# LariWa/Fractal-Image-Compression

Hardware: NVIDIA B200
Metric: encode_evals_per_s (higher is better)
Workload: dtype u8

## Files before the change

### fractal-image-compression_b200/csrc/fic_search_umma.cu

```cuda
#include <cuda_fp16.h>

#include <cmath>
#include <mutex>
#include <tuple>
#include <vector>

#include "fic_device.cuh"

namespace fic {

namespace {

constexpr int kTileN = 128;
constexpr int kBlockM = 128;
constexpr int kAccs = 4;
constexpr int kRowsPerSB = kBlockM * kAccs;
constexpr int kEpiWarps = 16;
constexpr int kThreads = (4 + kEpiWarps) * 32;
constexpr int kChunksPerTile = kTileN / 32;
constexpr int kBoundBytes = kChunksPerTile * 2 * 4 + 16 + kChunksPerTile * 4;
constexpr int kNormOff = kChunksPerTile * 2 * 4 + 16;
constexpr int kFlagLists = 2;
constexpr int kFlagCap = 32;
constexpr float kOneMinusEps = 1.0f - 1.9073486328125e-06f;

template <int B, bool F16>
struct Cfg;
template <>
struct Cfg<8, false> {
    static constexpr int n = 64;
    static constexpr int NB = 4;
    static constexpr bool KSPLIT = false;
    static constexpr int KS_A = 3;
    static constexpr int KS_B = 5;
    static constexpr int NS = 5;
    static constexpr int NSTAGE = 7;
    __host__ __device__ static constexpr int amap(int s) { return s < 4 ? (s & 1) : 2; }
    __host__ __device__ static constexpr bool is_l_slice(int s) { return s == 2 || s == 3; }
// ... 782 lines not shown
                            ((uint32_t)(kBlockM >> 4) << 24);
constexpr uint32_t kIdescF16 = (1u << 4) | (0u << 7) | (0u << 10) | ((uint32_t)(kTileN >> 3) << 17) |
                               ((uint32_t)(kBlockM >> 4) << 24);
constexpr uint32_t kIdescPair = (2u << 4) | (0u << 7) | (1u << 10) | ((uint32_t)(kTileN >> 3) << 17) |
                                ((uint32_t)((2 * kBlockM) >> 4) << 24);
constexpr uint32_t kIdescF16Pair = (1u << 4) | (0u << 7) | (0u << 10) | ((uint32_t)(kTileN >> 3) << 17) |
                                   ((uint32_t)((2 * kBlockM) >> 4) << 24);


template <int B, bool F16, bool PAIR>
__host__ __device__ constexpr int epi_of() { return (!F16 || B == 16) ? 0 : ((B == 4 || PAIR) ? 3 : 2); }

template <int B, bool F16, bool PAIR, bool DUMP>
__global__ void __launch_bounds__(kThreads, 1)
k_umma_search(const uint8_t *__restrict__ opA, const uint8_t *__restrict__ opB, const int32_t *__restrict__ vRarr,
              const float *__restrict__ nRarr, int2 *__restrict__ flag_list, int32_t *__restrict__ flag_cnt, uint32_t *__restrict__ row_lb, int n_sb,
              int n_chunks, int ntiles, int iso_shift, int64_t rows_padded, int32_t *__restrict__ dump, int64_t dump_ld, volatile int *status)
{
    using C = Cfg<B, F16>;
    using L = Lay<B, F16>;
    static_assert(!PAIR || F16 || C::KSPLIT, "CTA pairs: kind::f16, or the K-split configurations (B = 16)");
    constexpr int EPI = DUMP ? 0 : epi_of<B, F16, PAIR>();
    constexpr int NISS = (PAIR && !C::KSPLIT) ? 2 : 1;
    constexpr int NSTAGE = PAIR ? L::PAIR_STAGES : C::NSTAGE;
    constexpr int SLOT = PAIR ? L::PAIR_SLOT_BYTES : L::SLOT_BYTES;
    extern __shared__ __align__(1024) uint8_t smem_raw[];
    uint8_t *smem = (uint8_t *)(((uintptr_t)smem_raw + 1023) & ~(uintptr_t)1023);
    uint8_t *sA = smem;
    uint8_t *sB = smem + L::A_SB_BYTES;
    uint64_t *bars = (uint64_t *)(sB + C::NSTAGE * L::SLOT_BYTES);
    uint32_t bar0 = smem_u32(bars);
    asm volatile("" : "+r"(bar0));
    auto BAR_B_FULL = [&](int s) { return bar0 + 8u * s; };
    auto BAR_B_EMPTY = [&](int s) { return bar0 + 8u * (NSTAGE + s); };
    auto BAR_T_FULL = [&](int q) { return bar0 + 8u * (2 * NSTAGE + q); };
    auto BAR_T_EMPTY = [&](int q) { return bar0 + 8u * (2 * NSTAGE + kAccs + q); };
    const uint32_t BAR_A_FULL = bar0 + 8u * (2 * NSTAGE + 2 * kAccs);
    const uint32_t BAR_A_EMPTY = BAR_A_FULL + 8u;
    uint32_t *tmem_slot = (uint32_t *)(bars + 2 * NSTAGE + 2 * kAccs + 2);
    const uint32_t s_has_l = bar0 + 400u;
    uint32_t *s_lb = (uint32_t *)((uint8_t *)bars + L::BAR_BYTES);

    const int warp = threadIdx.x >> 5, lane = threadIdx.x & 31;
    const uint32_t rank = PAIR ? cluster_ctarank() : 0u;
    const int u_first = PAIR ? (int)(blockIdx.x >> 1) : (int)blockIdx.x, u_step = PAIR ? (int)(gridDim.x >> 1) : (int)gridDim.x;
    const int n_sbu = PAIR ? (n_sb >> 1) : n_sb;

    if (warp == 1 && lane == 0) {
        const uint32_t both = (PAIR && rank == 0) ? 2u : 1u;
        for (int s = 0; s < NSTAGE; s++) {
            mbar_init(BAR_B_FULL(s), both);
            mbar_init(BAR_B_EMPTY(s), NISS);
        }
        for (int q = 0; q < kAccs; q++) {
            mbar_init(BAR_T_FULL(q), 1);
            mbar_init(BAR_T_EMPTY(q), both * (kEpiWarps / kAccs));
        }
        mbar_init(BAR_A_FULL, both);
        mbar_init(BAR_A_EMPTY, NISS);
        asm volatile("fence.mbarrier_init.release.cluster;" ::: "memory");
    }
    if (warp == 2) {
        if (PAIR) {
            asm volatile("tcgen05.alloc.cta_group::2.sync.aligned.shared::cta.b32 [%0], %1;" ::"r"(smem_u32(tmem_slot)), "r"(512u) : "memory");
            asm volatile("tcgen05.relinquish_alloc_permit.cta_group::2.sync.aligned;" ::: "memory");
        } else {
            asm volatile("tcgen05.alloc.cta_group::1.sync.aligned.shared::cta.b32 [%0], %1;" ::"r"(smem_u32(tmem_slot)), "r"(512u) : "memory");
            asm volatile("tcgen05.relinquish_alloc_permit.cta_group::1.sync.aligned;" ::: "memory");
        }
    }
    tc_fence_before();
    if (PAIR) cluster_sync_all();
    else __syncthreads();
    tc_fence_after();
    const uint32_t tmem_base = *tmem_slot;

    const int n_units = n_sbu * n_chunks;

    if (warp == 0) {
        if (lane == 0) {
            uint32_t stage = 0, phase = 0, a_phase = 0;
            for (int u = u_first; u < n_units; u += u_step) {
                int sb = PAIR ? 2 * (u % n_sbu) + (int)rank : u % n_sbu, ch = u / n_sbu;
                int t0 = (int)((int64_t)ch * ntiles / n_chunks), t1 = (int)((int64_t)(ch + 1) * ntiles / n_chunks);
                mbar_wait(BAR_A_EMPTY, a_phase ^ 1, status, 1);
                mbar_expect_tx(BAR_A_FULL, L::A_SB_BYTES);
                bulk_g2s(smem_u32(sA), opA + (int64_t)sb * L::A_SB_BYTES, L::A_SB_BYTES, BAR_A_FULL);
                for (int t = t0; t < t1; t++) {
                    const uint8_t *blob = opB + (int64_t)t * L::B_TILE_BYTES;
                    if (C::KSPLIT && PAIR) {
                        const uint32_t has_l = __ldg((const uint32_t *)(blob + L::B_OP_BYTES + kChunksPerTile * 8));
                        mbar_wait(BAR_B_EMPTY(stage), phase ^ 1, status, 2);
                        sts_u32(s_has_l + 4u * stage, has_l);
                        mbar_expect_tx(BAR_B_FULL(stage), L::PAIR_P0_BYTES);
                        bulk_g2s(smem_u32(sB + stage * SLOT), blob + rank * L::PAIR_P0_BYTES, L::PAIR_P0_BYTES, BAR_B_FULL(stage));
                        if (++stage == NSTAGE) { stage = 0; phase ^= 1; }
                        if (has_l) {
                            mbar_wait(BAR_B_EMPTY(stage), phase ^ 1, status, 2);
                            mbar_expect_tx(BAR_B_FULL(stage), L::PAIR_P1_BYTES);
// ... 22 lines not shown
                        mbar_expect_tx(BAR_B_FULL(stage), L::B_TILE_BYTES);
                        bulk_g2s(smem_u32(sB + stage * L::SLOT_BYTES), blob, L::B_TILE_BYTES, BAR_B_FULL(stage));
                        if (++stage == NSTAGE) { stage = 0; phase ^= 1; }
                    }
                }
                a_phase ^= 1;
            }
        }
        __syncwarp();
    } else if (PAIR && (warp == 1 || (warp == 3 && !C::KSPLIT))) {
        if constexpr (PAIR && C::KSPLIT) {
            if (rank == 0) {
                uint32_t stage = 0, phase = 0, a_phase = 0, t_phase = 0;
                const uint32_t elected = elect_one();
                const uint64_t a_desc0 = make_desc(smem_u32(sA), 128, L::SBO_A);
                for (int u = u_first; u < n_units; u += u_step) {
                    int ch = u / n_sbu;
                    int t0 = (int)((int64_t)ch * ntiles / n_chunks), t1 = (int)((int64_t)(ch + 1) * ntiles / n_chunks);
                    mbar_wait(BAR_A_FULL, a_phase, status, 3);
                    for (int t = t0; t < t1; t++) {
                        mbar_wait(BAR_B_FULL(stage), phase, status, 4);
                        tc_fence_after();
                        const uint32_t has_l = lds_volatile_u32(s_has_l + 4u * stage);
                        const uint64_t b0 = make_desc(smem_u32(sB + stage * SLOT), 128, L::SBO_B);
#pragma unroll
                        for (int q = 0; q < C::NB; q++) {
                            mbar_wait(BAR_T_EMPTY(q), ((t_phase >> q) & 1) ^ 1, status, 5);
                            tc_fence_after();
                            if (elected) {
#pragma unroll
                                for (int s = 0; s < L::KS0; s++) {
                                    const uint64_t ad = a_desc0 + (uint64_t)((q * L::A_BLOCK_BYTES + s * 256) >> 4);
                                    if (F16) tc_mma2_f16(tmem_base + q * kTileN, ad, b0 + (uint64_t)((s * 256) >> 4), kIdescF16Pair, s > 0 ? 1u : 0u);
// ... 26 lines not shown
                                __syncwarp();
                            }
                            if (elected) tc_commit2(BAR_B_EMPTY(stage), 3u);
                            __syncwarp();
                            if (++stage == NSTAGE) { stage = 0; phase ^= 1; }
                        }
                    }
                    if (elected) tc_commit2(BAR_A_EMPTY, 3u);
                    __syncwarp();
                    a_phase ^= 1;
                }
            } else {
                if (lane == 0) {
                    uint32_t stage = 0, phase = 0, a_phase = 0;
                    const uint32_t ra_full = mapa_u32(BAR_A_FULL, 0);
                    for (int u = u_first; u < n_units; u += u_step) {
                        int ch = u / n_sbu;
                        int t0 = (int)((int64_t)ch * ntiles / n_chunks), t1 = (int)((int64_t)(ch + 1) * ntiles / n_chunks);
                        mbar_wait(BAR_A_FULL, a_phase, status, 3);
                        mbar_arrive_cluster(ra_full);
                        for (int t = t0; t < t1; t++) {
                            mbar_wait(BAR_B_FULL(stage), phase, status, 4);
                            const uint32_t has_l = lds_volatile_u32(s_has_l + 4u * stage);
                            mbar_arrive_cluster(mapa_u32(BAR_B_FULL(stage), 0));
                            if (++stage == NSTAGE) { stage = 0; phase ^= 1; }
                            if (has_l) {
                                mbar_wait(BAR_B_FULL(stage), phase, status, 4);
                                mbar_arrive_cluster(mapa_u32(BAR_B_FULL(stage), 0));
                                if (++stage == NSTAGE) { stage = 0; phase ^= 1; }
                            }
                        }
                        a_phase ^= 1;
                    }
                }
                __syncwarp();
            }
        } else if constexpr (PAIR) {
            if (rank == 0) {
                const int qi = warp >> 1;
                uint32_t stage = 0, phase = 0, a_phase = 0, t_phase = 0;
                const uint32_t elected = elect_one();
                const uint64_t a_desc0 = make_desc(smem_u32(sA), 128, L::SBO_A);
                const uint64_t b_desc0 = make_desc(smem_u32(sB), 128, L::SBO_B);
                for (int u = u_first; u < n_units; u += u_step) {
                    int ch = u / n_sbu;
                    int t0 = (int)((int64_t)ch * ntiles / n_chunks), t1 = (int)((int64_t)(ch + 1) * ntiles / n_chunks);
                    mbar_wait(BAR_A_FULL, a_phase, status, 3);
                    for (int t = t0; t < t1; t++) {
                        mbar_wait(BAR_B_FULL(stage), phase, status, 4);
                        tc_fence_after();
                        const uint64_t b_desc = b_desc0 + (uint64_t)((stage * SLOT) >> 4);
#pragma unroll
                        for (int k = 0; k < 2; k++) {
                            const int q = qi + 2 * k;
                            mbar_wait(BAR_T_EMPTY(q), ((t_phase >> k) & 1) ^ 1, status, 5);
                            tc_fence_after();
                            if (elected) {
#pragma unroll
                                for (int s = 0; s < C::NS; s++) {
                                    const uint64_t ad = a_desc0 + (uint64_t)((q * L::A_BLOCK_BYTES + C::amap(s) * 256) >> 4);
                                    tc_mma2_f16(tmem_base + q * kTileN, ad, b_desc + (uint64_t)((s * 256) >> 4), kIdescF16Pair, s > 0 ? 1u : 0u);
// ... 2 lines not shown
                                if (k == 1) tc_commit2(BAR_B_EMPTY(stage), 3u);
                            }
                            __syncwarp();
                            t_phase ^= 1u << k;
                        }
                        if (++stage == NSTAGE) { stage = 0; phase ^= 1; }
                    }
                    if (elected) tc_commit2(BAR_A_EMPTY, 3u);
                    __syncwarp();
                    a_phase ^= 1;
                }
            } else if (warp == 1) {
                if (lane == 0) {
                    uint32_t stage = 0, phase = 0, a_phase = 0;
                    const uint32_t ra_full = mapa_u32(BAR_A_FULL, 0);
                    for (int u = u_first; u < n_units; u += u_step) {
                        int ch = u / n_sbu;
                        int t0 = (int)((int64_t)ch * ntiles / n_chunks), t1 = (int)((int64_t)(ch + 1) * ntiles / n_chunks);
                        mbar_wait(BAR_A_FULL, a_phase, status, 3);
                        mbar_arrive_cluster(ra_full);
                        for (int t = t0; t < t1; t++) {
                            mbar_wait(BAR_B_FULL(stage), phase, status, 4);
                            mbar_arrive_cluster(mapa_u32(BAR_B_FULL(stage), 0));
                            if (++stage == NSTAGE) { stage = 0; phase ^= 1; }
                        }
                        a_phase ^= 1;
                    }
                }
                __syncwarp();
            }
        }
    } else if (warp == 1) {
        uint32_t stage = 0, phase = 0, a_phase = 0, t_phase = 0;
        const uint32_t elected = elect_one();
        const uint64_t a_desc0 = make_desc(smem_u32(sA), 128, L::SBO_A);
        const uint64_t b_desc0 = make_desc(smem_u32(sB), 128, L::SBO_B);
        for (int u = u_first; u < n_units; u += u_step) {
            int ch = u / n_sbu;
            int t0 = (int)((int64_t)ch * ntiles / n_chunks), t1 = (int)((int64_t)(ch + 1) * ntiles / n_chunks);
            mbar_wait(BAR_A_FULL, a_phase, status, 3);
            for (int t = t0; t < t1; t++) {
                mbar_wait(BAR_B_FULL(stage), phase, status, 4);
                tc_fence_after();
                const uint32_t has_l = *(volatile const uint32_t *)(sB + stage * L::SLOT_BYTES + L::B_OP_BYTES + kChunksPerTile * 8);
                if (C::KSPLIT) {
                    const uint64_t b0 = make_desc(smem_u32(sB + stage * L::SLOT_BYTES), 128, L::SBO_B);
#pragma unroll
                    for (int q = 0; q < C::NB; q++) {
                        mbar_wait(BAR_T_EMPTY(q), ((t_phase >> q) & 1) ^ 1, status, 5);
                        tc_fence_after();
                        if (elected) {
#pragma unroll
                            for (int s = 0; s < L::KS0; s++) {
                                const uint64_t ad = a_desc0 + (uint64_t)((q * L::A_BLOCK_BYTES + s * 256) >> 4);
// ... 58 lines not shown
            if (elected) tc_commit(BAR_A_EMPTY);
            __syncwarp();
            a_phase ^= 1;
        }
    } else if (warp >= 4) {
        const int e = warp - 4;
        const int lq = e & 3, q = e >> 2;
        const uint32_t ta = tmem_base + ((uint32_t)(lq * 32) << 16) + q * kTileN;
        uint32_t tf_phase = 0;
        const uint32_t bar_hand_back = PAIR ? mapa_u32(BAR_T_EMPTY(q), 0) : BAR_T_EMPTY(q);
        auto hand_back = [&]() {
            if (PAIR) mbar_arrive_cluster(bar_hand_back);
            else mbar_arrive(bar_hand_back);
        };
        constexpr bool SLACK = B == 16 && F16;
        const int n_units_mine = q < C::NB ? n_units : 0;
        for (int u = u_first; u < n_units_mine; u += u_step) {
            int sb = PAIR ? 2 * (u % n_sbu) + (int)rank : u % n_sbu, ch = u / n_sbu;
            int t0 = (int)((int64_t)ch * ntiles / n_chunks), t1 = (int)((int64_t)(ch + 1) * ntiles / n_chunks);
            const int64_t row = (int64_t)sb * L::ROWS_SB + q * kBlockM + lq * 32 + lane;
            const int vR = vRarr[row];
            const float nR = SLACK ? nRarr[row] : 0.0f;
            RowFilter st;
            st.thresh = (vR == 0) ? __int_as_float(0x7f800000) : -1.0f;
            st.lbmax = 0.0f;
            st.cnt = 0;
            const float tie_abs = (float)(vR * vR) * 4.76837158203125e-07f;
            const uint32_t sh_lb = smem_u32(s_lb + q * kBlockM + (((lq * 32 + lane) >> iso_shift) << iso_shift));
            if (iso_shift) {
                sts_u32(sh_lb, 0u);
                __syncwarp();
            }
            if (ch > 0 && vR != 0) {
                const float seed = __uint_as_float(*(volatile const uint32_t *)(row_lb + ((row >> iso_shift) << iso_shift)));
                if (seed > 0.0f) {
                    st.lbmax = seed;
                    st.thresh = flag_threshold(seed, tie_abs);
                }
            }
            int2 *const list0 = flag_list + (((int64_t)ch * rows_padded + row) * kFlagLists) * kFlagCap;
            int cnt0 = 0, cnt1 = 0;
            for (int t = t0; t < t1; t++) {
                const float4 *gb = (const float4 *)(opB + (int64_t)t * L::B_TILE_BYTES + L::B_OP_BYTES);
                const float4 bnd01 = __ldg(gb), bnd23 = __ldg(gb + 1);
                float4 bndn = make_float4(0.0f, 0.0f, 0.0f, 0.0f);
                if (SLACK) bndn = __ldg(gb + 3);
                mbar_wait(BAR_T_FULL(q), tf_phase, status, 7);
                tc_fence_after();
                if (iso_shift) {
                    const float other = __uint_as_float(lds_volatile_u32(sh_lb));
                    if (other > st.lbmax) {
                        st.lbmax = other;
                        st.thresh = flag_threshold(other, tie_abs);
                    }
                }
// ... 106 lines not shown
                            Mu = M + sl;
                            Ml = fmaxf(M - sl, 0.0f);
                        }
                    }
                    const float ub = Mu * rhi;
                    if (ub > st.thresh) {
                        st.cnt = c < 2 ? cnt0 : cnt1;
                        st = flag_chunk(st, Ml * rlo, ub, tie_abs, list0 + (c >> 1) * kFlagCap, t * kChunksPerTile + c, sh_lb, iso_shift ? 1 : 0);
                        if (c < 2) cnt0 = st.cnt;
                        else cnt1 = st.cnt;
                    }
                }
                }
                tf_phase ^= 1;
            }
            flag_cnt[((int64_t)ch * rows_padded + row) * 2] = cnt0;
            flag_cnt[((int64_t)ch * rows_padded + row) * 2 + 1] = cnt1;
            if (st.lbmax > 0.0f) atomicMax(row_lb + ((row >> iso_shift) << iso_shift), __float_as_uint(st.lbmax));
        }
    }

    tc_fence_before();
    if (PAIR) cluster_sync_all();
    else __syncthreads();
    if (warp == 2) {
        tc_fence_after();
        if (PAIR) asm volatile("tcgen05.dealloc.cta_group::2.sync.aligned.b32 %0, %1;" ::"r"(tmem_base), "r"(512u) : "memory");
        else asm volatile("tcgen05.dealloc.cta_group::1.sync.aligned.b32 %0, %1;" ::"r"(tmem_base), "r"(512u) : "memory");
    }
}


// ... 120 lines not shown
    constexpr int n = B * B;
    int kov = 0;
#pragma unroll
    for (int c = 0; c < n / 16; c++) {
        const uint4 d = __ldg((const uint4 *)(pos_raw + raw_offset<n>(pos, c)));
        const uint4 r = *(const uint4 *)(rw + 4 * c);
        kov = dp4a_uu(r.x, d.x, kov);
        kov = dp4a_uu(r.y, d.y, kov);
        kov = dp4a_uu(r.z, d.z, kov);
        kov = dp4a_uu(r.w, d.w, kov);
    }
    return kov - (rmean * dsum + (dsum / n) * vR);
}

template <class F>
__device__ __forceinline__ void for_each_flagged(int lane, int64_t i, int64_t rows_padded, int n_chunks, int64_t npos,
                                                 const int2 *__restrict__ flag_list, const int32_t *__restrict__ flag_cnt,
                                                 float th, F &&consider)
{
    const int n_lists = kFlagLists * n_chunks;
    const int my_cnt = lane < n_lists ? flag_cnt[((int64_t)(lane / kFlagLists) * rows_padded + i) * kFlagLists + (lane % kFlagLists)] : 0;
    const bool overflow = __any_sync(0xffffffffu, my_cnt > kFlagCap);
    if (!overflow) {
        for (int lh = 0; lh < n_lists; lh++) {
            const int cnt = __shfl_sync(0xffffffffu, my_cnt, lh);
            if (cnt == 0) continue;
            const int2 *lst = flag_list + (((int64_t)(lh / kFlagLists) * rows_padded + i) * kFlagLists + (lh % kFlagLists)) * kFlagCap;
            const int2 mine = lane < cnt ? lst[lane] : make_int2(0, 0);
            unsigned live = __ballot_sync(0xffffffffu, lane < cnt && __int_as_float(mine.y) > th);
            while (live) {
                const int e = __ffs(live) - 1;
                live &= live - 1;
                consider((int64_t)__shfl_sync(0xffffffffu, mine.x, e) * 32 + lane);
            }
        }
    } else {
        for (int64_t pos = lane; pos < npos; pos += 32) consider(pos);
    }
}

template <int B>
__global__ void __launch_bounds__(128)
k_umma_refine(const uint8_t *__restrict__ src, const int32_t *__restrict__ rsum, const uint8_t *__restrict__ pos_raw,
              const int4 *__restrict__ pos_info,
              const int2 *__restrict__ flag_list, const int32_t *__restrict__ flag_cnt,
              const uint32_t *__restrict__ row_lb, int n_chunks,
              int64_t rows_padded, int64_t rows, int64_t npos, const int64_t *__restrict__ dom0_pos,
              int32_t *__restrict__ best, Geom g, int64_t j0)
{
    constexpr int n = B * B;
    constexpr int NW = n / 4;
    const int warp = threadIdx.x >> 5, lane = threadIdx.x & 31;
    const int64_t i = (int64_t)blockIdx.x * 4 + warp;
    if (i >= rows) return;
    const int64_t j = j0 + i;
    int rmean;
    const int vR = centred_sum(rsum[j], n, &rmean);
    if (vR == 0) {
        if (lane == 0) best[j] = 0;
        return;
    }
// ... 25 lines not shown
    auto consider = [&](int64_t pos) {
        const int4 pi = __ldg(pos_info + pos);
        const int idx = pi.x;
        if (idx >= 0) {
            const int varD = pi.y;
            const int kov = refine_kov<B>(rw, rmean, vR, pos_raw, pos, pi.z);
            const float ax = varD > 0 ? fabsf((float)kov) * __frsqrt_rn((float)varD) : 0.0f;
            if (ax * (1.0f + 2.384185791015625e-07f) > th) {
                argmin_merge(be, bi, grey_error(kov, vR, __dsqrt_rn((double)varD)), idx);
                const float xlo = ax * (1.0f - 2.384185791015625e-07f);
                if (xlo > lb) { lb = xlo; th = flag_threshold(lb, tie_abs); }
            }
        }
    };
    if (lane == 0) consider(*dom0_pos);
    for_each_flagged(lane, i, rows_padded, n_chunks, npos, flag_list, flag_cnt, th_row, consider);
    warp_argmin(be, bi);
    if (lane == 0) best[j] = bi == 0x7fffffff ? 0 : bi;
}

template <int B>
__global__ void __launch_bounds__(128)
k_umma_refine_iso(const uint8_t *__restrict__ src, const int32_t *__restrict__ rsum, const uint8_t *__restrict__ pos_raw,
                  const int4 *__restrict__ pos_info, const int2 *__restrict__ flag_list,
                  const int32_t *__restrict__ flag_cnt, const uint32_t *__restrict__ row_lb, int n_chunks,
                  int64_t rows_padded, int64_t ranges, int64_t npos,
                  const int64_t *__restrict__ dom0_pos, int32_t *__restrict__ best, Geom g, int64_t j0)
{
    constexpr int n = B * B;
    constexpr int NW = n / 4;
    __shared__ uint8_t s_blk[4][n];
    const int warp = threadIdx.x >> 5, lane = threadIdx.x & 31;
    const int64_t r = (int64_t)blockIdx.x * 4 + warp;
    if (r >= ranges) return;
    const int64_t j = j0 + r;
    int rmean;
    const int vR = centred_sum(rsum[j], n, &rmean);
    if (vR == 0) {
        if (lane == 0) best[j] = 0;
        return;
// ... 28 lines not shown
        const int4 pi = __ldg(pos_info + pos);
        if (pi.x >= 0) {
            const int kov = refine_kov<B>(rw, rmean, vR, pos_raw, pos, pi.z);
            const float ax = pi.y > 0 ? fabsf((float)kov) * __frsqrt_rn((float)pi.y) : 0.0f;
            if (ax * (1.0f + 2.384185791015625e-07f) > th) {
                argmin_merge(be, bi, grey_error(kov, vR, __dsqrt_rn((double)pi.y)), pi.x * 8 + kiso);
                const float xlo = ax * (1.0f - 2.384185791015625e-07f);
                if (xlo > lb) { lb = xlo; th = flag_threshold(lb, tie_abs); }
            }
        }
    };
    build(0);
    if (lane == 0) consider(*dom0_pos, 0);
    int built = 0;
    bool overflow = false;
    for (int ch = 0; ch < n_chunks && !overflow; ch++) {
        const int64_t base = ((int64_t)ch * rows_padded + r * 8) * kFlagLists;
        const int my_cnt = lane < 8 * kFlagLists ? flag_cnt[base + lane] : 0;
        if (__any_sync(0xffffffffu, my_cnt > kFlagCap)) { overflow = true; break; }
        for (int kiso = 0; kiso < 8; kiso++) {
            int any = 0;
            for (int h = 0; h < kFlagLists; h++) any |= __shfl_sync(0xffffffffu, my_cnt, kFlagLists * kiso + h);
            if (any == 0) continue;
            if (built != kiso) { build(kiso); built = kiso; }
#pragma unroll 1
            for (int h = 0; h < kFlagLists; h++) {
                const int cnt = __shfl_sync(0xffffffffu, my_cnt, kFlagLists * kiso + h);
                if (cnt == 0) continue;
                const int2 *lst = flag_list + (base + kFlagLists * kiso + h) * kFlagCap;
                const int2 mine = lane < cnt ? lst[lane] : make_int2(0, 0);
                unsigned live = __ballot_sync(0xffffffffu, lane < cnt && __int_as_float(mine.y) > th_row);
// ... 7 lines not shown
    }
    if (overflow) {
        for (int kiso = 0; kiso < 8; kiso++) {
            build(kiso);
            for (int64_t pos = lane; pos < npos; pos += 32) consider(pos, kiso);
        }
    }
    warp_argmin(be, bi);
    if (lane == 0) best[j] = bi == 0x7fffffff ? 0 : bi;
}

template <int B>
__global__ void __launch_bounds__(128)
k_umma_refine_rgb(const uint8_t *__restrict__ src, const int32_t *__restrict__ rsum, const uint8_t *__restrict__ opB,
                  const int4 *__restrict__ pos_info, const int2 *__restrict__ flag_list, const int32_t *__restrict__ flag_cnt,
                  const uint32_t *__restrict__ row_lb, int n_chunks,
                  int64_t rows_padded, int64_t rows, int64_t npos, const int64_t *__restrict__ dom0_pos,
                  int32_t *__restrict__ best, Geom g, int64_t j0)
{
    using L = Lay<B, true>;
    constexpr int n = B * B;
    const int warp = threadIdx.x >> 5, lane = threadIdx.x & 31;
    const int64_t i = (int64_t)blockIdx.x * 4 + warp;
    if (i >= rows) return;
    const int64_t j = j0 + i;
    int rm[3];
    const int vRi = centred_sum_rgb(rsum, g.NR, j, n, rm);
    const int rmsum = rm[0] + rm[1] + rm[2];
    if (vRi == 0) {
        if (lane == 0) best[j] = 0;
        return;
// ... 29 lines not shown
                    const float2 f = __half22float2(*(const __half2 *)&w[e]);
                    kov = rgb_kov_step(kov, gR[c * 8 + 2 * e], f.x);
                    kov = rgb_kov_step(kov, gR[c * 8 + 2 * e + 1], f.y);
                }
            }
            const float vD = (float)pi.y;
            const float ax = pi.y > 0 ? __fdiv_rn(fabsf(kov), vD) : 0.0f;
            if (ax * (1.0f + 2.384185791015625e-07f) > th) {
                argmin_merge(be, bi, rgb_error(kov, vR, vD), idx);
                const float xlo = ax * (1.0f - 2.384185791015625e-07f);
                if (xlo > lb) { lb = xlo; th = flag_threshold(lb, tie_abs); }
            }
        }
    };
    if (lane == 0) consider(*dom0_pos);
    for_each_flagged(lane, i, rows_padded, n_chunks, npos, flag_list, flag_cnt, th_row, consider);
    warp_argmin(be, bi);
    if (lane == 0) best[j] = bi == 0x7fffffff ? 0 : bi;
}


inline int64_t pad_up(int64_t v, int64_t m) { return (v + m - 1) / m * m; }
inline uint64_t gcd_u64(uint64_t a, uint64_t b) { while (b) { uint64_t t = a % b; a = b; b = t; } return a; }

struct Plan {
    int64_t rp;
    int n_sb, ntiles, n_chunks;
    uint32_t mult;
    int64_t npos;
};

inline int rows_per_sb(const Geom &g) { return (g.C == 3 && g.B == 16 ? 2 : kAccs) * kBlockM; }

inline Plan make_plan(const Geom &g, int64_t rows, int num_sms)
{
    Plan p;
    const int rows_sb = rows_per_sb(g);
    p.rp = pad_up(rows, 2 * rows_sb);
    p.n_sb = (int)(p.rp / rows_sb);
    p.ntiles = (int)((g.ND + kTileN - 1) / kTileN);
    p.npos = (int64_t)p.ntiles * kTileN;
    p.n_chunks = 1;
    const double tile_s = (g.B == 16 ? (g.C == 3 ? 2300.0 : 4650.0) : (g.B == 8 ? 1550.0 : 1400.0)) / 1.9e9;
    const double flag_s = 0.11e-9 * (g.n / 64.0) * (g.n > 64 ? 0.7 : 1.0);
    double best_cost = 0;
    for (int c = 1; c <= 8 && c <= p.ntiles; c++) {
        const int64_t units = (int64_t)p.n_sb * c;
        const int64_t waves = (units + num_sms - 1) / num_sms;
        const double tiles_per_unit = (double)((p.ntiles + c - 1) / c);
        const double flags_per_row = 2.0 * (log(2.0 * tiles_per_unit) + 0.58) + 2.0 * (c - 1) * 1.5;
        const double cost = (double)waves * tiles_per_unit * tile_s + (double)rows * flags_per_row * flag_s;
        if (c == 1 || cost < best_cost * 0.98) { best_cost = cost; p.n_chunks = c; }
    }
    const uint64_t nch = (uint64_t)p.ntiles * kChunksPerTile;
    uint64_t m = (uint64_t)((double)nch * 0.6180339887498949) | 1u;
    while (gcd_u64(m, nch) != 1) m += 2;
    p.mult = nch <= 8 ? 1u : (uint32_t)(m % nch);
    return p;
}

template <int B, bool F16>
struct OpBLayout {
    size_t off_posdom, off_posinfo, off_posraw, off_dom0, off_keys0, off_keys1, off_vals0, off_vals1, off_temp,
        temp_bytes, total;
    OpBLayout(const Geom &g, const Plan &p)
    {
        size_t o = (size_t)p.ntiles * Lay<B, F16>::B_TILE_BYTES;
        auto take = [&](size_t bytes) { size_t at = (o + 255) & ~(size_t)255; o = at + bytes; return at; };
// ... 1 lines not shown
        off_posinfo = take((size_t)p.npos * 16);
        off_posraw = take((size_t)p.npos * (B * B));
        off_dom0 = take(16);
        off_keys0 = take((size_t)g.ND * 4);
        off_keys1 = take((size_t)g.ND * 4);
        off_vals0 = take((size_t)g.ND * 4);
        off_vals1 = take((size_t)g.ND * 4);
        temp_bytes = sort_hist_bytes(g.ND);
        off_temp = take(temp_bytes + 256);
        total = o + 256;
    }
};

template <int B, bool F16>
struct OpALayout {
    static constexpr int kCntSlots = 4;
    size_t off_vR, off_cnt, off_list, off_lb, off_norm, total;
    explicit OpALayout(const Plan &p)
    {
        off_vR = (size_t)p.n_sb * Lay<B, F16>::A_SB_BYTES;
        off_cnt = off_vR + (size_t)p.rp * 4;
        off_list = off_cnt + (size_t)p.rp * p.n_chunks * kCntSlots * 4;
        off_lb = off_list + (size_t)p.rp * p.n_chunks * kFlagLists * kFlagCap * sizeof(int2);
        off_norm = off_lb + (size_t)p.rp * 4;
        total = off_norm + (size_t)p.rp * 4 + 1024;
    }
};

template <int B, bool F16>
size_t opA_bytes_t(const Geom &g, int64_t rows, int num_sms)
{
    return OpALayout<B, F16>(make_plan(g, rows, num_sms)).total;
}

using KernelT = void (*)(const uint8_t *, const uint8_t *, const int32_t *, const float *, int2 *, int32_t *, uint32_t *, int, int,
                         int, int, int64_t, int32_t *, int64_t, volatile int *);

template <int B, bool F16>
constexpr bool pair_capable() { return F16 || B == 16; }
template <int B, bool F16>
constexpr bool pair_default() { return pair_capable<B, F16>() && B >= 8; }

inline bool pair_launchable(KernelT kern, int smem_bytes)
{
    static std::mutex mu;
    static std::vector<std::tuple<KernelT, int, bool>> known;
    int dev = 0;
    cudaGetDevice(&dev);
    {
        std::lock_guard<std::mutex> lock(mu);
        for (const auto &k : known)
// ... 71 lines not shown
    bool pair = false;
    KernelT kern = dump ? k_umma_search<B, F16, false, true> : k_umma_search<B, F16, false, false>;
    if constexpr (pair_capable<B, F16>()) {
        pair = (pair_mode == FIC_UMMA_PAIR_ON || (pair_mode != FIC_UMMA_PAIR_OFF && pair_default<B, F16>())) && num_sms >= 2;
        if (pair) {
            KernelT pk = dump ? k_umma_search<B, F16, true, true> : k_umma_search<B, F16, true, false>;
            ce = cudaFuncSetAttribute(pk, cudaFuncAttributeMaxDynamicSharedMemorySize, L::SMEM_BYTES);
            if (ce != cudaSuccess) { *err = cudaGetErrorString(ce); return -1; }
            if (pair_launchable(pk, L::SMEM_BYTES)) kern = pk;
            else pair = false;
        }
    }
    if (pair_used) *pair_used = pair ? 1 : 0;
    ce = cudaFuncSetAttribute(kern, cudaFuncAttributeMaxDynamicSharedMemorySize, L::SMEM_BYTES);
    if (ce != cudaSuccess) { *err = cudaGetErrorString(ce); return -1; }
    int n_units = pair ? (p.n_sb / 2) * p.n_chunks : p.n_sb * p.n_chunks;
    const int slots = pair ? num_sms / 2 : num_sms;
    int grid = (n_units < slots ? n_units : slots) * (pair ? 2 : 1);
    if (k0) cudaEventRecord(k0, s);
    cudaMemsetAsync(row_lb, 0, (size_t)rp * 4, s);
    {
        cudaLaunchConfig_t cfg = {};
        cfg.gridDim = dim3((unsigned)grid);
        cfg.blockDim = dim3(kThreads);
        cfg.dynamicSmemBytes = L::SMEM_BYTES;
        cfg.stream = s;
        cudaLaunchAttribute at[1];
        at[0].id = cudaLaunchAttributeClusterDimension;
        at[0].val.clusterDim.x = 2;
        at[0].val.clusterDim.y = 1;
        at[0].val.clusterDim.z = 1;
        cfg.attrs = at;
        cfg.numAttrs = pair ? 1 : 0;
        const uint8_t *opA_c = opA, *opB_c = w.opB;
        const int32_t *vR_c = vR;
        const float *norm_c = row_norm;
        const int iso_shift = g.n_iso > 1 ? 3 : 0;
        volatile int *status_v = status_dev;
        ce = cudaLaunchKernelEx(&cfg, kern, opA_c, opB_c, vR_c, norm_c, flag_list, flag_cnt, row_lb, p.n_sb, p.n_chunks, p.ntiles, iso_shift,
                                rp, dump, dump_ld, status_v);
        if (ce != cudaSuccess) { *err = cudaGetErrorString(ce); return -1; }
    }
    if (k1) cudaEventRecord(k1, s);
    if (rgb) {
        if constexpr (F16)
            k_umma_refine_rgb<B><<<(unsigned)((rows + 3) / 4), 128, 0, s>>>(w.src, w.rsum, w.opB, pos_info, flag_list, flag_cnt,
                                                                            row_lb, p.n_chunks, rp, rows, p.npos, dom0, w.best, g, j0);
    } else if (g.n_iso > 1)
        k_umma_refine_iso<B><<<(unsigned)((j1 - j0 + 3) / 4), 128, 0, s>>>(w.src, w.rsum, pos_raw, pos_info, flag_list, flag_cnt,
                                                                         row_lb, p.n_chunks, rp, j1 - j0, p.npos, dom0, w.best, g, j0);
    else
        k_umma_refine<B><<<(unsigned)((rows + 3) / 4), 128, 0, s>>>(w.src, w.rsum, pos_raw, pos_info, flag_list, flag_cnt,
                                                                    row_lb, p.n_chunks, rp, rows, p.npos, dom0, w.best, g, j0);
    launches += 2;
    ce = cudaGetLastError();
    if (ce != cudaSuccess) { *err = cudaGetErrorString(ce); return -1; }
    return launches;
}

#define FIC_UMMA_DISPATCH(B_, F_, EXPR_I8_4, EXPR_I8_8, EXPR_I8_16, EXPR_F16_4, EXPR_F16_8, EXPR_F16_16) \
    ((B_) == 16 ? ((F_) ? (EXPR_F16_16) : (EXPR_I8_16)) : ((F_) ? ((B_) == 8 ? (EXPR_F16_8) : (EXPR_F16_4)) : ((B_) == 8 ? (EXPR_I8_8) : (EXPR_I8_4))))

}

int umma_default_kind(const Geom &g) { return g.B == 16 ? FIC_UMMA_KIND_I8 : FIC_UMMA_KIND_F16; }

static bool use_f16(const Geom &g, int kind)
{
// ... 251 lines not shown
```

Before: 13090.

## Split tail work units across idle SMs to balance the last wave

Replaces the round-robin assignment of (superblock, chunk) units to persistent CTAs with a UnitSplit scheduler. Whole waves are assigned as before, and the leftover units of the final partial wave are cut into tile-range pieces spread over more slots. Partial pieces write to extra flag-list sets, so the layout gains n_sets lists and the refine kernels iterate over n_sets. The extra counters are zeroed with a memset. This targets wave-quantization idle SMs, at the cost of more flag storage, extra A reloads, and more lists to scan in refine.

```diff
diff --git a/fractal-image-compression_b200/csrc/fic_search_umma.cu b/fractal-image-compression_b200/csrc/fic_search_umma.cu
--- a/fractal-image-compression_b200/csrc/fic_search_umma.cu
+++ b/fractal-image-compression_b200/csrc/fic_search_umma.cu
@@ -1,5 +1,6 @@
 #include <cuda_fp16.h>
 
+#include <algorithm>
 #include <cmath>
 #include <mutex>
 #include <tuple>
@@ -22,6 +23,61 @@
 constexpr int kNormOff = kChunksPerTile * 2 * 4 + 16;
 constexpr int kFlagLists = 2;
 constexpr int kFlagCap = 32;
+constexpr int kMaxSets = 32 / kFlagLists;
+constexpr int kMinPiece = 4;
+
+struct UnitSplit {
+    int n_sbu, n_chunks, ntiles, slots, tail_slots;
+    struct Item { int su, ch, set, t0, t1; };
+    __host__ __device__ int tile0(int ch) const { return (int)((int64_t)ch * ntiles / n_chunks); }
+    __host__ __device__ int64_t start(int u) const
+    {
+        const int ch = u / n_sbu;
+        return (int64_t)n_sbu * tile0(ch) + (int64_t)(u - ch * n_sbu) * (tile0(ch + 1) - tile0(ch));
+    }
+    __host__ __device__ int unit_at(int64_t x) const
+    {
+        int ch = n_chunks - 1;
+        while (ch > 0 && (int64_t)n_sbu * tile0(ch) > x) ch--;
+        const int64_t len = tile0(ch + 1) - tile0(ch);
+        return ch * n_sbu + (int)((x - (int64_t)n_sbu * tile0(ch)) / len);
+    }
+    __host__ __device__ int whole() const { return tail_slots ? n_sbu * n_chunks / slots : (n_sbu * n_chunks + slots - 1) / slots; }
+    __host__ __device__ int64_t piece(int k) const
+    {
+        const int64_t tail0 = start(whole() * slots), T = start(n_sbu * n_chunks) - tail0;
+        return tail0 + T * k / tail_slots;
+    }
+    __host__ __device__ int piece_of(int64_t x) const
+    {
+        const int64_t tail0 = start(whole() * slots), T = start(n_sbu * n_chunks) - tail0;
+        return (int)(((x - tail0 + 1) * tail_slots - 1) / T);
+    }
+    __host__ __device__ bool item(int slot, int it, Item &w) const
+    {
+        const int W = whole(), n_units = n_sbu * n_chunks;
+        const int u = it < W ? slot + it * slots : (slot < tail_slots ? unit_at(piece(slot)) + (it - W) : n_units);
+        if (u >= n_units) return false;
+        w.su = u % n_sbu;
+        w.ch = u / n_sbu;
+        w.t0 = tile0(w.ch);
+        w.t1 = tile0(w.ch + 1);
+        w.set = w.ch;
+        if (it >= W) {
+            const int64_t s = start(u), e = start(u + 1), p0 = piece(slot), p1 = piece(slot + 1);
+            const int64_t lo = it == W ? p0 : s, hi = p1 < e ? p1 : e;
+            if (lo >= hi) return false;
+            if (lo > s) {
+                int j = slot - piece_of(s);
+                for (int v = u - n_sbu; v >= W * slots; v -= n_sbu) j += piece_of(start(v + 1) - 1) - piece_of(start(v));
+                w.set = n_chunks + j - 1;
+            }
+            w.t0 += (int)(lo - s);
+            w.t1 = w.t0 + (int)(hi - lo);
+        }
+        return true;
+    }
+};
 constexpr float kOneMinusEps = 1.0f - 1.9073486328125e-06f;
 
 template <int B, bool F16>
@@ -834,8 +890,8 @@
 template <int B, bool F16, bool PAIR, bool DUMP>
 __global__ void __launch_bounds__(kThreads, 1)
 k_umma_search(const uint8_t *__restrict__ opA, const uint8_t *__restrict__ opB, const int32_t *__restrict__ vRarr,
-              const float *__restrict__ nRarr, int2 *__restrict__ flag_list, int32_t *__restrict__ flag_cnt, uint32_t *__restrict__ row_lb, int n_sb,
-              int n_chunks, int ntiles, int iso_shift, int64_t rows_padded, int32_t *__restrict__ dump, int64_t dump_ld, volatile int *status)
+              const float *__restrict__ nRarr, int2 *__restrict__ flag_list, int32_t *__restrict__ flag_cnt, uint32_t *__restrict__ row_lb, UnitSplit split,
+              int iso_shift, int64_t rows_padded, int32_t *__restrict__ dump, int64_t dump_ld, volatile int *status)
 {
     using C = Cfg<B, F16>;
     using L = Lay<B, F16>;
@@ -863,8 +919,7 @@
 
     const int warp = threadIdx.x >> 5, lane = threadIdx.x & 31;
     const uint32_t rank = PAIR ? cluster_ctarank() : 0u;
-    const int u_first = PAIR ? (int)(blockIdx.x >> 1) : (int)blockIdx.x, u_step = PAIR ? (int)(gridDim.x >> 1) : (int)gridDim.x;
-    const int n_sbu = PAIR ? (n_sb >> 1) : n_sb;
+    const int slot = PAIR ? (int)(blockIdx.x >> 1) : (int)blockIdx.x;
 
     if (warp == 1 && lane == 0) {
         const uint32_t both = (PAIR && rank == 0) ? 2u : 1u;
@@ -895,14 +950,12 @@
     tc_fence_after();
     const uint32_t tmem_base = *tmem_slot;
 
-    const int n_units = n_sbu * n_chunks;
-
     if (warp == 0) {
         if (lane == 0) {
             uint32_t stage = 0, phase = 0, a_phase = 0;
-            for (int u = u_first; u < n_units; u += u_step) {
-                int sb = PAIR ? 2 * (u % n_sbu) + (int)rank : u % n_sbu, ch = u / n_sbu;
-                int t0 = (int)((int64_t)ch * ntiles / n_chunks), t1 = (int)((int64_t)(ch + 1) * ntiles / n_chunks);
+            UnitSplit::Item wi;
+            for (int it = 0; split.item(slot, it, wi); it++) {
+                const int sb = PAIR ? 2 * wi.su + (int)rank : wi.su, t0 = wi.t0, t1 = wi.t1;
                 mbar_wait(BAR_A_EMPTY, a_phase ^ 1, status, 1);
                 mbar_expect_tx(BAR_A_FULL, L::A_SB_BYTES);
                 bulk_g2s(smem_u32(sA), opA + (int64_t)sb * L::A_SB_BYTES, L::A_SB_BYTES, BAR_A_FULL);
@@ -955,9 +1008,9 @@
                 uint32_t stage = 0, phase = 0, a_phase = 0, t_phase = 0;
                 const uint32_t elected = elect_one();
                 const uint64_t a_desc0 = make_desc(smem_u32(sA), 128, L::SBO_A);
-                for (int u = u_first; u < n_units; u += u_step) {
-                    int ch = u / n_sbu;
-                    int t0 = (int)((int64_t)ch * ntiles / n_chunks), t1 = (int)((int64_t)(ch + 1) * ntiles / n_chunks);
+                UnitSplit::Item wi;
+                for (int it = 0; split.item(slot, it, wi); it++) {
+                    const int t0 = wi.t0, t1 = wi.t1;
                     mbar_wait(BAR_A_FULL, a_phase, status, 3);
                     for (int t = t0; t < t1; t++) {
                         mbar_wait(BAR_B_FULL(stage), phase, status, 4);
@@ -1014,9 +1067,9 @@
                 if (lane == 0) {
                     uint32_t stage = 0, phase = 0, a_phase = 0;
                     const uint32_t ra_full = mapa_u32(BAR_A_FULL, 0);
-                    for (int u = u_first; u < n_units; u += u_step) {
-                        int ch = u / n_sbu;
-                        int t0 = (int)((int64_t)ch * ntiles / n_chunks), t1 = (int)((int64_t)(ch + 1) * ntiles / n_chunks);
+                    UnitSplit::Item wi;
+                    for (int it = 0; split.item(slot, it, wi); it++) {
+                        const int t0 = wi.t0, t1 = wi.t1;
                         mbar_wait(BAR_A_FULL, a_phase, status, 3);
                         mbar_arrive_cluster(ra_full);
                         for (int t = t0; t < t1; t++) {
@@ -1042,9 +1095,9 @@
                 const uint32_t elected = elect_one();
                 const uint64_t a_desc0 = make_desc(smem_u32(sA), 128, L::SBO_A);
                 const uint64_t b_desc0 = make_desc(smem_u32(sB), 128, L::SBO_B);
-                for (int u = u_first; u < n_units; u += u_step) {
-                    int ch = u / n_sbu;
-                    int t0 = (int)((int64_t)ch * ntiles / n_chunks), t1 = (int)((int64_t)(ch + 1) * ntiles / n_chunks);
+                UnitSplit::Item wi;
+                for (int it = 0; split.item(slot, it, wi); it++) {
+                    const int t0 = wi.t0, t1 = wi.t1;
                     mbar_wait(BAR_A_FULL, a_phase, status, 3);
                     for (int t = t0; t < t1; t++) {
                         mbar_wait(BAR_B_FULL(stage), phase, status, 4);
@@ -1077,9 +1130,9 @@
                 if (lane == 0) {
                     uint32_t stage = 0, phase = 0, a_phase = 0;
                     const uint32_t ra_full = mapa_u32(BAR_A_FULL, 0);
-                    for (int u = u_first; u < n_units; u += u_step) {
-                        int ch = u / n_sbu;
-                        int t0 = (int)((int64_t)ch * ntiles / n_chunks), t1 = (int)((int64_t)(ch + 1) * ntiles / n_chunks);
+                    UnitSplit::Item wi;
+                    for (int it = 0; split.item(slot, it, wi); it++) {
+                        const int t0 = wi.t0, t1 = wi.t1;
                         mbar_wait(BAR_A_FULL, a_phase, status, 3);
                         mbar_arrive_cluster(ra_full);
                         for (int t = t0; t < t1; t++) {
@@ -1098,9 +1151,9 @@
         const uint32_t elected = elect_one();
         const uint64_t a_desc0 = make_desc(smem_u32(sA), 128, L::SBO_A);
         const uint64_t b_desc0 = make_desc(smem_u32(sB), 128, L::SBO_B);
-        for (int u = u_first; u < n_units; u += u_step) {
-            int ch = u / n_sbu;
-            int t0 = (int)((int64_t)ch * ntiles / n_chunks), t1 = (int)((int64_t)(ch + 1) * ntiles / n_chunks);
+        UnitSplit::Item wi;
+        for (int it = 0; split.item(slot, it, wi); it++) {
+            const int t0 = wi.t0, t1 = wi.t1;
             mbar_wait(BAR_A_FULL, a_phase, status, 3);
             for (int t = t0; t < t1; t++) {
                 mbar_wait(BAR_B_FULL(stage), phase, status, 4);
@@ -1189,10 +1242,9 @@
             else mbar_arrive(bar_hand_back);
         };
         constexpr bool SLACK = B == 16 && F16;
-        const int n_units_mine = q < C::NB ? n_units : 0;
-        for (int u = u_first; u < n_units_mine; u += u_step) {
-            int sb = PAIR ? 2 * (u % n_sbu) + (int)rank : u % n_sbu, ch = u / n_sbu;
-            int t0 = (int)((int64_t)ch * ntiles / n_chunks), t1 = (int)((int64_t)(ch + 1) * ntiles / n_chunks);
+        UnitSplit::Item wi;
+        for (int it = 0; q < C::NB && split.item(slot, it, wi); it++) {
+            const int sb = PAIR ? 2 * wi.su + (int)rank : wi.su, ch = wi.ch, t0 = wi.t0, t1 = wi.t1;
             const int64_t row = (int64_t)sb * L::ROWS_SB + q * kBlockM + lq * 32 + lane;
             const int vR = vRarr[row];
             const float nR = SLACK ? nRarr[row] : 0.0f;
@@ -1213,7 +1265,7 @@
                     st.thresh = flag_threshold(seed, tie_abs);
                 }
             }
-            int2 *const list0 = flag_list + (((int64_t)ch * rows_padded + row) * kFlagLists) * kFlagCap;
+            int2 *const list0 = flag_list + (((int64_t)wi.set * rows_padded + row) * kFlagLists) * kFlagCap;
             int cnt0 = 0, cnt1 = 0;
             for (int t = t0; t < t1; t++) {
                 const float4 *gb = (const float4 *)(opB + (int64_t)t * L::B_TILE_BYTES + L::B_OP_BYTES);
@@ -1350,8 +1402,8 @@
                 }
                 tf_phase ^= 1;
             }
-            flag_cnt[((int64_t)ch * rows_padded + row) * 2] = cnt0;
-            flag_cnt[((int64_t)ch * rows_padded + row) * 2 + 1] = cnt1;
+            flag_cnt[((int64_t)wi.set * rows_padded + row) * 2] = cnt0;
+            flag_cnt[((int64_t)wi.set * rows_padded + row) * 2 + 1] = cnt1;
             if (st.lbmax > 0.0f) atomicMax(row_lb + ((row >> iso_shift) << iso_shift), __float_as_uint(st.lbmax));
         }
     }
@@ -1502,11 +1554,11 @@
 }
 
 template <class F>
-__device__ __forceinline__ void for_each_flagged(int lane, int64_t i, int64_t rows_padded, int n_chunks, int64_t npos,
+__device__ __forceinline__ void for_each_flagged(int lane, int64_t i, int64_t rows_padded, int n_sets, int64_t npos,
                                                  const int2 *__restrict__ flag_list, const int32_t *__restrict__ flag_cnt,
                                                  float th, F &&consider)
 {
-    const int n_lists = kFlagLists * n_chunks;
+    const int n_lists = kFlagLists * n_sets;
     const int my_cnt = lane < n_lists ? flag_cnt[((int64_t)(lane / kFlagLists) * rows_padded + i) * kFlagLists + (lane % kFlagLists)] : 0;
     const bool overflow = __any_sync(0xffffffffu, my_cnt > kFlagCap);
     if (!overflow) {
@@ -1532,7 +1584,7 @@
 k_umma_refine(const uint8_t *__restrict__ src, const int32_t *__restrict__ rsum, const uint8_t *__restrict__ pos_raw,
               const int4 *__restrict__ pos_info,
               const int2 *__restrict__ flag_list, const int32_t *__restrict__ flag_cnt,
-              const uint32_t *__restrict__ row_lb, int n_chunks,
+              const uint32_t *__restrict__ row_lb, int n_sets,
               int64_t rows_padded, int64_t rows, int64_t npos, const int64_t *__restrict__ dom0_pos,
               int32_t *__restrict__ best, Geom g, int64_t j0)
 {
@@ -1588,7 +1640,7 @@
         }
     };
     if (lane == 0) consider(*dom0_pos);
-    for_each_flagged(lane, i, rows_padded, n_chunks, npos, flag_list, flag_cnt, th_row, consider);
+    for_each_flagged(lane, i, rows_padded, n_sets, npos, flag_list, flag_cnt, th_row, consider);
     warp_argmin(be, bi);
     if (lane == 0) best[j] = bi == 0x7fffffff ? 0 : bi;
 }
@@ -1597,7 +1649,7 @@
 __global__ void __launch_bounds__(128)
 k_umma_refine_iso(const uint8_t *__restrict__ src, const int32_t *__restrict__ rsum, const uint8_t *__restrict__ pos_raw,
                   const int4 *__restrict__ pos_info, const int2 *__restrict__ flag_list,
-                  const int32_t *__restrict__ flag_cnt, const uint32_t *__restrict__ row_lb, int n_chunks,
+                  const int32_t *__restrict__ flag_cnt, const uint32_t *__restrict__ row_lb, int n_sets,
                   int64_t rows_padded, int64_t ranges, int64_t npos,
                   const int64_t *__restrict__ dom0_pos, int32_t *__restrict__ best, Geom g, int64_t j0)
 {
@@ -1656,7 +1708,7 @@
     if (lane == 0) consider(*dom0_pos, 0);
     int built = 0;
     bool overflow = false;
-    for (int ch = 0; ch < n_chunks && !overflow; ch++) {
+    for (int ch = 0; ch < n_sets && !overflow; ch++) {
         const int64_t base = ((int64_t)ch * rows_padded + r * 8) * kFlagLists;
         const int my_cnt = lane < 8 * kFlagLists ? flag_cnt[base + lane] : 0;
         if (__any_sync(0xffffffffu, my_cnt > kFlagCap)) { overflow = true; break; }
@@ -1694,7 +1746,7 @@
 __global__ void __launch_bounds__(128)
 k_umma_refine_rgb(const uint8_t *__restrict__ src, const int32_t *__restrict__ rsum, const uint8_t *__restrict__ opB,
                   const int4 *__restrict__ pos_info, const int2 *__restrict__ flag_list, const int32_t *__restrict__ flag_cnt,
-                  const uint32_t *__restrict__ row_lb, int n_chunks,
+                  const uint32_t *__restrict__ row_lb, int n_sets,
                   int64_t rows_padded, int64_t rows, int64_t npos, const int64_t *__restrict__ dom0_pos,
                   int32_t *__restrict__ best, Geom g, int64_t j0)
 {
@@ -1754,7 +1806,7 @@
         }
     };
     if (lane == 0) consider(*dom0_pos);
-    for_each_flagged(lane, i, rows_padded, n_chunks, npos, flag_list, flag_cnt, th_row, consider);
+    for_each_flagged(lane, i, rows_padded, n_sets, npos, flag_list, flag_cnt, th_row, consider);
     warp_argmin(be, bi);
     if (lane == 0) best[j] = bi == 0x7fffffff ? 0 : bi;
 }
@@ -1766,9 +1818,42 @@
 struct Plan {
     int64_t rp;
     int n_sb, ntiles, n_chunks;
+    int n_sets;
+    UnitSplit one, two;
     uint32_t mult;
     int64_t npos;
 };
+
+inline int sets_of(const UnitSplit &s)
+{
+    int m = s.n_chunks;
+    UnitSplit::Item w;
+    for (int k = 0; k < s.tail_slots; k++)
+        for (int it = s.whole(); s.item(k, it, w); it++) m = w.set + 1 > m ? w.set + 1 : m;
+    return m;
+}
+
+inline UnitSplit split_units(int n_sbu, int n_chunks, int ntiles, int slots)
+{
+    UnitSplit s{n_sbu, n_chunks, ntiles, slots < 1 ? 1 : slots, 0};
+    if ((n_sbu * n_chunks) % s.slots == 0) return s;
+    s.tail_slots = 1;
+    const int64_t tail = s.start(n_sbu * n_chunks) - s.start(s.whole() * s.slots);
+    const int64_t most = std::max<int64_t>(n_sbu * n_chunks - s.whole() * s.slots, tail / kMinPiece);
+    for (int ts = (int)std::min<int64_t>(s.slots, most); ts > 0; ts--) {
+        s.tail_slots = ts;
+        if (sets_of(s) <= kMaxSets) return s;
+    }
+    s.tail_slots = 0;
+    return s;
+}
+
+inline int slots_used(const UnitSplit &s)
+{
+    const int n_units = s.n_sbu * s.n_chunks;
+    if (s.tail_slots == 0) return n_units < s.slots ? n_units : s.slots;
+    return s.whole() > 0 ? s.slots : s.tail_slots;
+}
 
 inline int rows_per_sb(const Geom &g) { return (g.C == 3 && g.B == 16 ? 2 : kAccs) * kBlockM; }
 
@@ -1792,6 +1877,9 @@
         const double cost = (double)waves * tiles_per_unit * tile_s + (double)rows * flags_per_row * flag_s;
         if (c == 1 || cost < best_cost * 0.98) { best_cost = cost; p.n_chunks = c; }
     }
+    p.one = split_units(p.n_sb, p.n_chunks, p.ntiles, num_sms);
+    p.two = split_units(p.n_sb / 2, p.n_chunks, p.ntiles, num_sms / 2);
+    p.n_sets = std::max(sets_of(p.one), sets_of(p.two));
     const uint64_t nch = (uint64_t)p.ntiles * kChunksPerTile;
     uint64_t m = (uint64_t)((double)nch * 0.6180339887498949) | 1u;
     while (gcd_u64(m, nch) != 1) m += 2;
@@ -1823,14 +1911,13 @@
 
 template <int B, bool F16>
 struct OpALayout {
-    static constexpr int kCntSlots = 4;
     size_t off_vR, off_cnt, off_list, off_lb, off_norm, total;
     explicit OpALayout(const Plan &p)
     {
         off_vR = (size_t)p.n_sb * Lay<B, F16>::A_SB_BYTES;
-        off_cnt = off_vR + (size_t)p.rp * 4;
-        off_list = off_cnt + (size_t)p.rp * p.n_chunks * kCntSlots * 4;
-        off_lb = off_list + (size_t)p.rp * p.n_chunks * kFlagLists * kFlagCap * sizeof(int2);
+        off_list = off_vR + (size_t)p.rp * 4;
+        off_cnt = off_list + (size_t)p.rp * p.n_sets * kFlagLists * kFlagCap * sizeof(int2);
+        off_lb = off_cnt + (size_t)p.rp * p.n_sets * kFlagLists * 4;
         off_norm = off_lb + (size_t)p.rp * 4;
         total = off_norm + (size_t)p.rp * 4 + 1024;
     }
@@ -1842,8 +1929,8 @@
     return OpALayout<B, F16>(make_plan(g, rows, num_sms)).total;
 }
 
-using KernelT = void (*)(const uint8_t *, const uint8_t *, const int32_t *, const float *, int2 *, int32_t *, uint32_t *, int, int,
-                         int, int, int64_t, int32_t *, int64_t, volatile int *);
+using KernelT = void (*)(const uint8_t *, const uint8_t *, const int32_t *, const float *, int2 *, int32_t *, uint32_t *, UnitSplit,
+                         int, int64_t, int32_t *, int64_t, volatile int *);
 
 template <int B, bool F16>
 constexpr bool pair_capable() { return F16 || B == 16; }
@@ -1945,11 +2032,11 @@
     if (pair_used) *pair_used = pair ? 1 : 0;
     ce = cudaFuncSetAttribute(kern, cudaFuncAttributeMaxDynamicSharedMemorySize, L::SMEM_BYTES);
     if (ce != cudaSuccess) { *err = cudaGetErrorString(ce); return -1; }
-    int n_units = pair ? (p.n_sb / 2) * p.n_chunks : p.n_sb * p.n_chunks;
-    const int slots = pair ? num_sms / 2 : num_sms;
-    int grid = (n_units < slots ? n_units : slots) * (pair ? 2 : 1);
+    const UnitSplit split = pair ? p.two : p.one;
+    const int grid = slots_used(split) * (pair ? 2 : 1);
     if (k0) cudaEventRecord(k0, s);
-    cudaMemsetAsync(row_lb, 0, (size_t)rp * 4, s);
+    int32_t *extra_cnt = flag_cnt + (int64_t)p.n_chunks * rp * kFlagLists;
+    cudaMemsetAsync(extra_cnt, 0, (size_t)((uint8_t *)(row_lb + rp) - (uint8_t *)extra_cnt), s);
     {
         cudaLaunchConfig_t cfg = {};
         cfg.gridDim = dim3((unsigned)grid);
@@ -1968,7 +2055,7 @@
         const float *norm_c = row_norm;
         const int iso_shift = g.n_iso > 1 ? 3 : 0;
         volatile int *status_v = status_dev;
-        ce = cudaLaunchKernelEx(&cfg, kern, opA_c, opB_c, vR_c, norm_c, flag_list, flag_cnt, row_lb, p.n_sb, p.n_chunks, p.ntiles, iso_shift,
+        ce = cudaLaunchKernelEx(&cfg, kern, opA_c, opB_c, vR_c, norm_c, flag_list, flag_cnt, row_lb, split, iso_shift,
                                 rp, dump, dump_ld, status_v);
         if (ce != cudaSuccess) { *err = cudaGetErrorString(ce); return -1; }
     }
@@ -1976,13 +2063,13 @@
     if (rgb) {
         if constexpr (F16)
             k_umma_refine_rgb<B><<<(unsigned)((rows + 3) / 4), 128, 0, s>>>(w.src, w.rsum, w.opB, pos_info, flag_list, flag_cnt,
-                                                                            row_lb, p.n_chunks, rp, rows, p.npos, dom0, w.best, g, j0);
+                                                                            row_lb, p.n_sets, rp, rows, p.npos, dom0, w.best, g, j0);
     } else if (g.n_iso > 1)
         k_umma_refine_iso<B><<<(unsigned)((j1 - j0 + 3) / 4), 128, 0, s>>>(w.src, w.rsum, pos_raw, pos_info, flag_list, flag_cnt,
-                                                                         row_lb, p.n_chunks, rp, j1 - j0, p.npos, dom0, w.best, g, j0);
+                                                                         row_lb, p.n_sets, rp, j1 - j0, p.npos, dom0, w.best, g, j0);
     else
         k_umma_refine<B><<<(unsigned)((rows + 3) / 4), 128, 0, s>>>(w.src, w.rsum, pos_raw, pos_info, flag_list, flag_cnt,
-                                                                    row_lb, p.n_chunks, rp, rows, p.npos, dom0, w.best, g, j0);
+                                                                    row_lb, p.n_sets, rp, rows, p.npos, dom0, w.best, g, j0);
     launches += 2;
     ce = cudaGetLastError();
     if (ce != cudaSuccess) { *err = cudaGetErrorString(ce); return -1; }
```

Measured after the change: 11980, median of 6. 0.915x the previous value.
